# kopacja/rho2sdf.jl

Hardware: AMD Instinct MI355X
Metric: Mvoxels/s SDF extract on 512^3 grid over 100k HEX8; max|err| vs ref (higher is better)
Workload: dtype f64

## Files before the change

### rho2sdf.jl_amd/csrc/r2s_device_math.hpp

```cpp
#pragma once
#include <hip/hip_runtime.h>
#include <stdint.h>

namespace r2s {

#define R2S_DEV __device__ __forceinline__

struct alignas(16) ElemRec {
    double X[8][3];
    double r[8];
    double mn[3];
    double mx[3];
    double rmax;
    double rmin;
    double C[8][3];
    double Cr[8];
    double pn[6][3];
    double po[6];
    double pi[6];
    double nw[10];
};

struct alignas(16) BandItem {
    int32_t imin[3];
// ... 1309 lines not shown
    s.alpha *= 0.5;
    s.ls += 1;
    if (s.ls == 30) s.phase = FS_UPD;
}

template <class ER>
R2S_DEV void iso_full_upd(const ER& E, double rt, double rtol, IsoFullLane& s)
{
    s.Delta = (s.alpha < 1.0) ? ((s.alpha > 0.0) ? s.alpha * s.dmax : 0.25 * s.dmax) : fmin(2.0, fmax(s.Delta, 2.0 * s.dmax));
    if (s.stop == 2) {
        const bool near_feas = (fabs(s.c) <= 1e4 * rtol);
        double xr[3];
        if (!near_feas && s.nrest < R2S_ISO_MAX_RESTORE && iso_restore(E, s.x, rt, s.xi, s.c, xr)) {
            s.xi[0] = xr[0]; s.xi[1] = xr[1]; s.xi[2] = xr[2];
            s.mu = 0.0; s.Delta = 2.0; s.pat = 0; s.nrest++;
            s.it += 1;
            if (s.it == R2S_ISO_MAXIT) iso_full_fail(s); else s.phase = FS_EVAL;
            return;
        }
        iso_full_fail(s);
        return;
    }
    if (s.stop == 3 || s.stop == 4) { s.phase = FS_DONE; return; }
#pragma unroll
    for (int i = 0; i < 3; ++i) s.xi[i] = fmin(fmax(fma(s.alpha, s.d[i], s.xi[i]), -1.0), 1.0);
    if (s.stop == 1) { s.phase = FS_DONE; return; }
    s.it += 1;
    if (s.it == R2S_ISO_MAXIT) iso_full_fail(s); else s.phase = FS_EVAL;
}

#ifndef R2S_ISO_FAST_IT
#define R2S_ISO_FAST_IT 16
#endif
enum { ISO_IDLE = 0, ISO_EVAL, ISO_QP, ISO_FINISH, ISO_DONE, ISO_BAIL };

struct IsoLane {
    double x[3];
    double xi[3], mu, Delta;
    Sym3 H;
    double a[3], g[3], d[3];
    double se;
    double f, c, lam_new;
    int pat, it, p, step, phase;
    bool corner;
    bool seen;
};

R2S_DEV void iso_lane_bounds(const IsoLane& s, double lo[3], double hi[3])
{
#pragma unroll
    for (int i = 0; i < 3; ++i) {
        lo[i] = fmax(-1.0 - s.xi[i], -s.Delta);
        hi[i] = fmin(1.0 - s.xi[i], s.Delta);
    }
}

R2S_DEV void iso_lane_start(IsoLane& s, const double x[3])
{
    s.x[0] = x[0]; s.x[1] = x[1]; s.x[2] = x[2];
    s.xi[0] = s.xi[1] = s.xi[2] = 0.0;
    s.mu = 0.0; s.Delta = 2.0;
    s.pat = 0; s.it = 0;
    s.seen = false;
    s.phase = ISO_EVAL;
}

template <class ER>
R2S_DEV void iso_lane_eval(const ER& E, double rt, double rtol, IsoLane& s)
{
    double r[3], J[3][3], G[3][3], M2[3][3];
#pragma unroll
    for (int i = 0; i < 3; ++i) {
        const TriEval t = tri_eval_full(R2S_CX(E, i), s.xi);
        r[i] = s.x[i] - t.v;
        J[i][0] = t.d1; J[i][1] = t.d2; J[i][2] = t.d3;
        M2[i][0] = t.m12; M2[i][1] = t.m13; M2[i][2] = t.m23;
    }
    const double f = dot3(r[0], r[1], r[2], r[0], r[1], r[2]);
    const TriEval tr = tri_eval_full(R2S_CR(E), s.xi);
    double c = tr.v - rt;
    s.a[0] = tr.d1; s.a[1] = tr.d2; s.a[2] = tr.d3;
    if (fabs(c) <= rtol) c = 0.0;
#pragma unroll
    for (int j = 0; j < 3; ++j)
        if (fabs(s.a[j]) <= rtol) s.a[j] = 0.0;
#pragma unroll
    for (int j = 0; j < 3; ++j) s.g[j] = -2.0 * dot3(r[0], r[1], r[2], J[0][j], J[1][j], J[2][j]);
#pragma unroll
    for (int i = 0; i < 3; ++i)
#pragma unroll
        for (int j = i; j < 3; ++j)
            G[i][j] = G[j][i] = 2.0 * dot3(J[0][i], J[1][i], J[2][i], J[0][j], J[1][j], J[2][j]);
    s.pat = iso_clean_pattern(s.pat, s.xi);
    double lam;
    {
        double num = 0.0, den = 0.0;
        const int sp[3] = {s.pat & 3, (s.pat >> 2) & 3, s.pat >> 4};
#pragma unroll
        for (int i = 0; i < 3; ++i)
            if (!sp[i]) { num = fma(s.a[i], s.g[i], num); den = fma(s.a[i], s.a[i], den); }
        lam = (den > 0.0) ? -num / den : 0.0;
    }
    double S[3];
    {
        const double mr[3] = {tr.m12, tr.m13, tr.m23};
#pragma unroll
        for (int q = 0; q < 3; ++q)
            S[q] = fma(lam, mr[q], -2.0 * dot3(r[0], r[1], r[2], M2[0][q], M2[1][q], M2[2][q]));
    }
    double lo[3], hi[3];
    iso_lane_bounds(s, lo, hi);
    const double e = -c;
    double mplus = 0.0, mminus = 0.0;
// ... 35 lines not shown
    } else {
        double gp[3];
        iso_qp_data(G, S, s.a, s.g, sigma, e, s.H, gp);
        s.se = sigma * e;
        s.p = s.pat;
        s.step = 0;
        s.phase = iso_face_spd(s.H, s.pat) ? ISO_QP : ISO_BAIL;
    }
}

R2S_DEV void iso_lane_qp(IsoLane& s)
{
    QpOut o;
    double lo[3], hi[3], gp[3];
    iso_lane_bounds(s, lo, hi);
#pragma unroll
    for (int i = 0; i < 3; ++i) gp[i] = fma(-s.se, s.a[i], s.g[i]);
    const double e = -s.c;
    const int rc = qp_pattern(s.p, s.H, gp, s.a, e, lo, hi, o);
    if (rc == 1 && o.kkt) {
#pragma unroll
        for (int i = 0; i < 3; ++i) s.d[i] = fmin(fmax(o.d[i], lo[i]), hi[i]);
        s.lam_new = o.lam;
        s.phase = ISO_FINISH;
    } else if (rc == 0) {
        s.phase = ISO_BAIL;
    } else {
        s.p = o.next;
        s.step += 1;
        if (!(s.step < R2S_QP_WALK && s.p >= 0)) s.phase = ISO_BAIL;
    }
}

template <class ER>
R2S_DEV void iso_lane_finish(const ER& E, double rt, double rtol, IsoLane& s)
{
    const double dmax = fmax(fabs(s.d[0]), fmax(fabs(s.d[1]), fabs(s.d[2])));
    const bool near_feas = (fabs(s.c) <= 1e4 * rtol);
    if (!(dmax > R2S_ISO_TOL)) {
        if (s.corner && !near_feas) { s.phase = ISO_BAIL; return; }
    } else {
        const double ad = dot3(s.a[0], s.a[1], s.a[2], s.d[0], s.d[1], s.d[2]);
        const double pred_c = fabs(s.c) - fabs(s.c + ad);
        const double gd = dot3(s.g[0], s.g[1], s.g[2], s.d[0], s.d[1], s.d[2]);
        const double mu_keep = (fabs(s.c) <= 1e10 * rtol) ? 0.5 : 1.0;
        double mu_t = s.corner ? s.mu : fmax(mu_keep * s.mu, 2.0 * fabs(s.lam_new));
        if (s.corner && pred_c > 0.0) {
            const double need = 2.0 * fma(0.5, s.se, gd) / pred_c;
            if (need > mu_t) mu_t = need;
        }
        if (!(fma(-mu_t, pred_c, gd) < 0.0)) {
            if (pred_c > 0.0) mu_t = 2.0 * gd / pred_c;
            else {
                s.phase = (near_feas && !s.corner) ? ISO_DONE : ISO_BAIL;
                return;
            }
        }
        const double D = fma(-mu_t, pred_c, gd);
        const double phi0 = fma(mu_t, fabs(s.c), s.f);
        double xt[3], ft, ct;
#pragma unroll
        for (int i = 0; i < 3; ++i) xt[i] = fmin(fmax(fma(1.0, s.d[i], s.xi[i]), -1.0), 1.0);
        iso_eval_fc(E, s.x, rt, xt, ft, ct);
        if (!(fma(mu_t, fabs(ct), ft) <= fma(1e-4 * 1.0, D, phi0))) { s.phase = ISO_BAIL; return; }
        s.mu = mu_t;
        s.Delta = fmin(2.0, fmax(s.Delta, 2.0 * dmax));
        if (!s.corner) s.pat = s.p;
        s.seen = s.seen || (s.c == 0.0);
#pragma unroll
        for (int i = 0; i < 3; ++i) s.xi[i] = xt[i];
        s.it += 1;
        s.phase = (s.it == R2S_ISO_FAST_IT) ? ISO_BAIL : ISO_EVAL;
        return;
    }
    s.Delta = fmin(2.0, fmax(s.Delta, 2.0 * dmax));
#pragma unroll
    for (int i = 0; i < 3; ++i) s.xi[i] = fmin(fmax(fma(1.0, s.d[i], s.xi[i]), -1.0), 1.0);
    s.phase = ISO_DONE;
}

struct VoxState {
    double cur;
    double xp[3];
};

R2S_DEV bool write_value(VoxState& s, double d, const double xp[3], bool sym = false)
{
    if (sym && fabs(d) == s.cur) {
        const bool less = xp[0] < s.xp[0] || (xp[0] == s.xp[0] && (xp[1] < s.xp[1] || (xp[1] == s.xp[1] && xp[2] < s.xp[2])));
        if (less) { s.xp[0] = xp[0]; s.xp[1] = xp[1]; s.xp[2] = xp[2]; }
        return false;
    }
    if (fabs(d) < s.cur) {
        s.cur = d;
        s.xp[0] = xp[0]; s.xp[1] = xp[1]; s.xp[2] = xp[2];
        return true;
    }
    return false;
}

R2S_DEV bool projected_on_full_segment(VoxState& s, const ElemRec& E, double rt, const double xp[3],
                                       const double x[3], bool sym = false)
{
    double xi[3], N[8];
    inv_map_hex8(E, xp, xi);
// ... 391 lines not shown
```

### rho2sdf.jl_amd/csrc/rho2sdf_hip.hip

```cpp
#include <hip/hip_runtime.h>

#include <algorithm>
#include <cmath>
#include <cstdarg>
#include <cstddef>
#include <cstdio>
#include <cstring>
#include <initializer_list>
#include <utility>
#include <string>
#include <vector>

#include "../../include/rho2sdf_hip.h"
#include "r2s_common.hpp"
#include "r2s_device_math.hpp"

#include <type_traits>

using namespace r2s;

__constant__ int c_hex_isn[6][4] = {{0, 3, 2, 1}, {0, 1, 5, 4}, {1, 2, 6, 5},
                                    {2, 3, 7, 6}, {3, 0, 4, 7}, {4, 5, 6, 7}};

#define SCAN_BLOCK 256
// ... 1055 lines not shown
                    c = seg_end;
                    if (next >= v_end) continue;
                }
                if (s.phase == ISO_IDLE) {
                    const uint32_t v = next + __builtin_amdgcn_mbcnt_hi((uint32_t)(m_idle >> 32),
                                                  __builtin_amdgcn_mbcnt_lo((uint32_t)m_idle, 0u));
                    if (v < v_end) {
                        uint32_t li, lj, lk;
                        box_decode(dec, v, li, lj, lk);
                        const int i = lo0 + (int)li, j = lo1 + (int)lj, kl = lo2 + (int)lk;
                        double x[3];
                        x[0] = grid_coord(g, 0, i);
                        x[1] = grid_coord(g, 1, j);
                        x[2] = grid_coord(g, 2, slab_global_k(sl, kl));
                        iso_lane_start(s, x);
#ifdef R2S_ISO_STATS
                        dbg_trips = 0; dbg_qp = 0; dbg_ls = 0; dbg_el = items[it].el;
#endif
                        my = tile_slot(st_off, tb, i, j, kl);
                        eslot = cur_slot;
                    }
                }
                next += (uint32_t)__popcll(m_idle);
            }
            if (exhausted && __ballot(s.phase != ISO_IDLE) == 0) {
#ifdef R2S_ISO_WAVE_END
                if (lane == 0 && blockIdx.x < 4094) g_iso_wave_end[blockIdx.x] = wall_clock64();
#endif
                break;
            }
        }
        {
            const IsoElemLds& E = slots[eslot];
            ISO_STAT(0, s.phase == ISO_EVAL)
            if (s.phase == ISO_EVAL) iso_lane_eval(E, rho_t, E.rtol, s);
            ISO_STAT(1, s.phase == ISO_QP)
            if (s.phase == ISO_QP) iso_lane_qp(s);
            if (__popcll(__ballot(s.phase == ISO_QP)) >= R2S_ISO_QP2_MIN) {
                ISO_STAT(7, s.phase == ISO_QP)
                if (s.phase == ISO_QP) iso_lane_qp(s);
            }
            ISO_STAT(2, s.phase == ISO_FINISH)
            if (s.phase == ISO_FINISH) iso_lane_finish(E, rho_t, E.rtol, s);
            ISO_STAT(5, true)
#ifdef R2S_ISO_STATS
            if (s.phase != ISO_IDLE) dbg_trips += 1;
#endif
        }
    }
}

#ifdef R2S_STRAG_DIAG
__device__ unsigned long long g_strag_diag[3 * 16384];
extern "C" int r2s_debug_strag_diag(unsigned long long* out)
{
    if (hipMemcpyFromSymbol(out, HIP_SYMBOL(g_strag_diag), sizeof(unsigned long long) * 3 * 16384) != hipSuccess) return 1;
    static unsigned long long z[3 * 16384];
    return hipMemcpyToSymbol(HIP_SYMBOL(g_strag_diag), z, sizeof z) != hipSuccess;
}
__device__ unsigned long long g_strag_hist[256];
extern "C" int r2s_debug_strag_hist(unsigned long long* out)
{
    if (hipMemcpyFromSymbol(out, HIP_SYMBOL(g_strag_hist), sizeof(unsigned long long) * 256) != hipSuccess) return 1;
    static unsigned long long z[256];
    return hipMemcpyToSymbol(HIP_SYMBOL(g_strag_hist), z, sizeof z) != hipSuccess;
}
#endif
struct IsoCoefPad {
    double C[8][3];
    double Cr[8];
    double pad;
};
#ifndef R2S_STRAG_REFILL_MIN
#define R2S_STRAG_REFILL_MIN 8
#endif
#ifndef R2S_ENUM_COOP_MAX
// ... 457 lines not shown
    }
}

__global__ void __launch_bounds__(256) fill_kernel(double* __restrict__ p, int64_t n, double v)
{
    const int64_t stride = (int64_t)gridDim.x * blockDim.x;
    int64_t i = (int64_t)blockIdx.x * blockDim.x + threadIdx.x;
    const int64_t n2 = n >> 1;
    double2* p2 = reinterpret_cast<double2*>(p);
    const double2 vv = make_double2(v, v);
    for (int64_t j = i; j < n2; j += stride) p2[j] = vv;
    if (i == 0 && (n & 1)) p[n - 1] = v;
}

struct MainArgs {
    GridDev g;
    SlabInfo s;
    double rho_t;
    const uint32_t* active;
    uint32_t n_active;
    const uint32_t* band_off;
    const uint32_t* band_ent;
    const uint32_t* sign_off;
    const uint32_t* sign_ent;
    const BandItem* items;
    const void* erec;
    double* dist;
    double* sign;
    double* sdf;
    double* xp;
    const double* iso_res;
    const double* iso_res_xp;
    const void* sbox;
    const uint32_t* s_store_off;
    const double* sres;
    const uint8_t* hot;
    const uint32_t* abort_flag;
    int true_min;
    int sdf_mode;
};

template <class Rec, bool DO_DIST, bool DO_SIGN, bool TRI = true, bool SYM = false>
__global__ void __launch_bounds__(256) sdf_tiles_kernel(MainArgs A)
{
    const Rec* __restrict__ erec = static_cast<const Rec*>(A.erec);
    const uint32_t w = __builtin_amdgcn_readfirstlane((blockIdx.x * blockDim.x + threadIdx.x) >> 6);
    if (w >= A.n_active) return;
    const int lane = threadIdx.x & 63;
    const uint32_t ab = *A.abort_flag;
    const uint32_t t = A.active[w];
    if (ab) return;
    const int tx = t % A.s.ntx, ty = (t / A.s.ntx) % A.s.nty, tz = t / (A.s.ntx * A.s.nty);
    const int i = tx * 4 + (lane & 3), j = ty * 4 + ((lane >> 2) & 3), kl = tz * 4 + (lane >> 4);
    const int k = slab_global_k(A.s, kl);
    const bool valid = (i < A.g.nx) && (j < A.g.ny) && (kl < A.s.nzl) && (k < A.s.k1);
    double x[3];
    x[0] = grid_coord(A.g, 0, i);
    x[1] = grid_coord(A.g, 1, j);
    x[2] = grid_coord(A.g, 2, k);

    VoxState st;
    st.cur = 1.0e10;
    st.xp[0] = st.xp[1] = st.xp[2] = 0.0;
    if (DO_DIST) {
        const int ci = (int)cell_of(A.g, 0, x[0]), cj = (int)cell_of(A.g, 1, x[1]),
                  ck = (int)cell_of(A.g, 2, x[2]);
        const uint32_t b = A.band_off[t], e = A.band_off[t + 1];
// ... 47 lines not shown
                                if (A.iso_res_xp) {
                                    st.xp[0] = A.iso_res_xp[3 * slot[u]];
                                    st.xp[1] = A.iso_res_xp[3 * slot[u] + 1];
                                    st.xp[2] = A.iso_res_xp[3 * slot[u] + 2];
                                }
                            }
                        } else if constexpr (TRI) {
                            const BandItem& T = A.items[__builtin_amdgcn_readlane(my_it, (int)(q0 + u))];
                            process_triangle<Rec, SYM>(st, T, erec[T.el], A.rho_t, x);
                        }
                    }
                }
            }
        }
    }
    double sg = -1.0;
    if (DO_SIGN) {
        const uint32_t b = A.sign_off[t], e = A.sign_off[t + 1];
        if constexpr (std::is_same<Rec, ElemRec>::value) {
            if (A.hot[t]) {
                const SignBox* __restrict__ sbox = static_cast<const SignBox*>(A.sbox);
                bool any = false, done = false;
                double cmax = -INFINITY, max_local = 10.0;
                for (uint32_t p0 = b; p0 < e; p0 += 64u) {
                    const uint32_t n = (e - p0 < 64u) ? e - p0 : 64u;
                    int32_t hs[9];
#pragma unroll
                    for (int q = 0; q < 9; ++q) hs[q] = 0;
                    if ((uint32_t)lane < n) {
                        const uint32_t el = A.sign_ent[p0 + lane];
                        const int32_t* w = reinterpret_cast<const int32_t*>(&sbox[el]);
#pragma unroll
                        for (int q = 0; q < 8; ++q) hs[q] = w[q];
                        hs[8] = (int32_t)A.s_store_off[el];
                    }
                    for (uint32_t q0 = 0; q0 < n; q0 += 4u) {
                        bool in[4];
                        double v[4], rmax[4];
#pragma unroll
                        for (int u = 0; u < 4; ++u) {
                            const bool ok = q0 + u < n;
                            const int qq = (int)(ok ? q0 + u : n - 1u);
                            int32_t hh[9];
#pragma unroll
                            for (int q = 0; q < 9; ++q) hh[q] = __builtin_amdgcn_readlane(hs[q], qq);
                            const int32_t lo3[3] = {hh[0], hh[1], hh[2]}, dim3[3] = {hh[3], hh[4], hh[5]};
                            const uint32_t di = (uint32_t)(i - lo3[0]), dj = (uint32_t)(j - lo3[1]), dk = (uint32_t)(kl - lo3[2]);
                            in[u] = valid && ok && di < (uint32_t)dim3[0] && dj < (uint32_t)dim3[1] && dk < (uint32_t)dim3[2];
                            rmax[u] = __hiloint2double(hh[7], hh[6]);
                            v[u] = INFINITY;
                            if (in[u] && !done)
                                v[u] = A.sres[(size_t)tile_chunk((uint32_t)hh[8], tile_box(lo3, dim3), tx, ty, tz) * 64u + (uint32_t)lane];
                        }
#pragma unroll
                        for (int u = 0; u < 4; ++u) {
                            if (in[u]) {
                                any = true;
                                if (rmax[u] > cmax) cmax = rmax[u];
                                const double m = fabs(v[u]);
                                if (A.true_min) {
                                    if (m < 1.01 && !__builtin_signbit(v[u])) sg = 1.0;
                                } else if (!done && m < 1.01 && max_local > m) {
                                    if (!__builtin_signbit(v[u])) sg = 1.0;
                                    if (m < 0.95) done = true;
                                    else max_local = m;
                                }
                            }
// ... 128 lines not shown
    const int lane = threadIdx.x & 63;
    const int ntx = (nx + 3) / 4, nty = (ny + 3) / 4;
    const uint32_t t = ids[w];
    const int tx = t % ntx, ty = (t / ntx) % nty, tz = t / (ntx * nty);
    const int i = tx * 4 + (lane & 3), j = ty * 4 + ((lane >> 2) & 3), k = tz * 4 + (lane >> 4);
    if (i < nx && j < ny && k < nz) volume[((int64_t)k * ny + j) * nx + i] = payload[(size_t)w * 64 + lane];
}
__global__ void __launch_bounds__(256) unpack_segments_masks_kernel(const double* __restrict__ buf, int64_t seglen, uint32_t cap_full,
                                                                   uint32_t cap_mask, int nx, int ny, int nz, double magnitude,
                                                                   double* __restrict__ volume)
{
    const double* __restrict__ seg = buf + (int64_t)blockIdx.y * seglen;
    const int64_t nf = reinterpret_cast<const int64_t*>(seg)[0], nm = reinterpret_cast<const int64_t*>(seg)[1];
    const uint32_t w = __builtin_amdgcn_readfirstlane((blockIdx.x * blockDim.x + threadIdx.x) >> 6);
    if (nf < 0 || nf > (int64_t)cap_full || nm < 0 || nm > (int64_t)cap_mask || (int64_t)w >= nm) return;
    const uint64_t* __restrict__ masks = reinterpret_cast<const uint64_t*>(seg + 2 + (int64_t)cap_full * 64 + (cap_full + 1) / 2);
    const uint32_t* __restrict__ ids = reinterpret_cast<const uint32_t*>(masks + cap_mask);
    const int lane = threadIdx.x & 63;
    const int ntx = (nx + 3) / 4, nty = (ny + 3) / 4;
    const uint32_t t = ids[w];
    const int tx = t % ntx, ty = (t / ntx) % nty, tz = t / (ntx * nty);
    const int i = tx * 4 + (lane & 3), j = ty * 4 + ((lane >> 2) & 3), k = tz * 4 + (lane >> 4);
    if (i < nx && j < ny && k < nz) volume[((int64_t)k * ny + j) * nx + i] = ((masks[w] >> lane) & 1ull) ? magnitude : -magnitude;
}

struct r2s_plan {
    int device = 0;
    int n_cu = 256;
    DevBuf deg, ine_ptr, ine, cursor, erec, cls, fmask, nitems, item_off, items;
    DevBuf band_cnt, band_off, band_raw, band_ent, sign_cnt, sign_off, sign_raw, sign_ent;
    DevBuf active, active_sign, active_any, active_sonly, active_lean, active_tri, tri, hot, counters, scan_tmp[3], scan_tmp2[3], nchunks, chunk_off, iso_res, iso_res_xp, strag;
    DevBuf perm, wchunks, hardflag;
    DevBuf sbox, s_nchunks, s_chunk_off, sres;
    DevBuf nstore, store_off, s_nstore, s_store_off;
    SlabInfo last_s;
    GridDev last_g;
    uint32_t last_n_any = 0, last_n_band = 0, last_n_sonly = 0;
    bool has_last = false;
    uint32_t* h_pinned = nullptr;
    uint32_t* d_pinned = nullptr;
    struct Spec {
        bool valid = false;
        int64_t key[12] = {0};
        uint32_t v[16] = {0};
    } spec;
    hipEvent_t ev[8] = {nullptr, nullptr, nullptr, nullptr, nullptr, nullptr, nullptr, nullptr};
    hipStream_t st2 = nullptr;
    hipStream_t st3 = nullptr;
    hipEvent_t ev2[8] = {nullptr, nullptr, nullptr, nullptr, nullptr, nullptr, nullptr, nullptr};
    hipEvent_t ev_fast[2] = {nullptr, nullptr};
    bool fast_timed = false;
};

static int scan_exclusive2(r2s_plan* P, const uint32_t* in0, uint32_t* out0, const uint32_t* in1, uint32_t* out1,
                           int64_t n, hipStream_t st, int level = 0, int bank = 0)
{
    DevBuf* tmp = bank ? P->scan_tmp2 : P->scan_tmp;
    if (n <= 0) return 0;
    const unsigned ny = in1 ? 2u : 1u;
    const int64_t nb = (n + SCAN_TILE - 1) / SCAN_TILE;
    ScanPair sp;
    sp.in[0] = in0; sp.out[0] = out0; sp.in[1] = in1; sp.out[1] = out1;
    sp.sums[0] = sp.sums[1] = nullptr;
    if (nb == 1) {
        scan_block_kernel<<<dim3(1, ny), SCAN_BLOCK, 0, st>>>(sp, n);
        return 0;
    }
// ... 107 lines not shown
    int rc = check_device(device);
    if (rc) return rc;
    HIP_TRY(hipSetDevice(device));
    r2s_plan* P = new r2s_plan();
    P->device = device;
    {
        hipDeviceProp_t prop;
        if (hipGetDeviceProperties(&prop, device) == hipSuccess && prop.multiProcessorCount > 0) P->n_cu = prop.multiProcessorCount;
    }
    HIP_TRY(hipHostMalloc((void**)&P->h_pinned, 128, hipHostMallocMapped | hipHostMallocCoherent));
    HIP_TRY(hipHostGetDevicePointer((void**)&P->d_pinned, P->h_pinned, 0));
    for (int i = 0; i < 8; ++i) HIP_TRY(hipEventCreate(&P->ev[i]));
    for (int i = 0; i < 8; ++i) HIP_TRY(hipEventCreate(&P->ev2[i]));
    for (int i = 0; i < 2; ++i) HIP_TRY(hipEventCreate(&P->ev_fast[i]));
    {
        int prio_lo = 0, prio_hi = 0;
        HIP_TRY(hipDeviceGetStreamPriorityRange(&prio_lo, &prio_hi));
        (void)prio_lo;
        HIP_TRY(hipStreamCreateWithPriority(&P->st2, hipStreamNonBlocking, prio_hi));
        HIP_TRY(hipStreamCreateWithFlags(&P->st3, hipStreamNonBlocking));
    }
    *out = P;
    return 0;
}

void r2s_plan_destroy(r2s_plan* P)
{
    if (!P) return;
    (void)hipSetDevice(P->device);
    DevBuf* all[] = {&P->deg, &P->ine_ptr, &P->ine, &P->cursor, &P->erec, &P->cls, &P->fmask, &P->nitems,
                     &P->item_off, &P->items, &P->band_cnt, &P->band_off, &P->band_raw, &P->band_ent,
                     &P->sign_cnt, &P->sign_off, &P->sign_raw, &P->sign_ent, &P->active, &P->active_sign, &P->active_any, &P->active_sonly, &P->active_lean, &P->active_tri, &P->tri,
                     &P->hot, &P->counters, &P->nchunks, &P->chunk_off, &P->iso_res, &P->iso_res_xp, &P->strag,
                     &P->perm, &P->wchunks, &P->hardflag, &P->sbox, &P->s_nchunks, &P->s_chunk_off, &P->sres, &P->nstore, &P->store_off, &P->s_nstore, &P->s_store_off,
                     &P->scan_tmp[0], &P->scan_tmp[1], &P->scan_tmp[2], &P->scan_tmp2[0], &P->scan_tmp2[1], &P->scan_tmp2[2]};
    for (DevBuf* b : all) b->release();
    if (P->h_pinned) (void)hipHostFree(P->h_pinned);
    for (int i = 0; i < 8; ++i)
        if (P->ev[i]) (void)hipEventDestroy(P->ev[i]);
    for (int i = 0; i < 8; ++i)
        if (P->ev2[i]) (void)hipEventDestroy(P->ev2[i]);
    for (int i = 0; i < 2; ++i)
        if (P->ev_fast[i]) (void)hipEventDestroy(P->ev_fast[i]);
    if (P->st2) (void)hipStreamDestroy(P->st2);
    if (P->st3) (void)hipStreamDestroy(P->st3);
    delete P;
}


}

static uint32_t iso_straggler_cap(uint32_t n_store)
{
    static const int cap_env = getenv("R2S_ISO_STRAGGLER_CAP") ? atoi(getenv("R2S_ISO_STRAGGLER_CAP")) : 0;
    if (cap_env > 0) return (uint32_t)cap_env;
    const uint64_t slots = 64ull * std::max<uint32_t>(n_store, 1u);
    return (uint32_t)std::max<uint64_t>(slots / 16, std::min<uint64_t>(slots, 1ull << 20));
}

static int iso_project_hex(r2s_plan* P, hipStream_t st, uint32_t n_items, uint32_t n_chunks, uint32_t n_store, uint32_t wps,
                           const GridDev& g, const SlabInfo& s, double rho_t, double* res_xp, uint32_t* counters,
                           const uint32_t* abort_flag)
{
    static const int free_env = getenv("R2S_ISO_FREE") ? atoi(getenv("R2S_ISO_FREE")) : 0;
    const uint32_t resident = (uint32_t)P->n_cu * 4u * wps - (uint32_t)std::min(std::max(free_env, 0), (int)P->n_cu * 4);
    static const int group_env = getenv("R2S_ISO_GROUP") ? atoi(getenv("R2S_ISO_GROUP")) : 0;
    const uint32_t group = group_env > 0 ? (uint32_t)group_env
// ... 128 lines not shown
    HIP_TRY(hipEventRecord(P->ev2[5], st));
    HIP_TRY(hipStreamWaitEvent(P->st2, P->ev2[0], 0));
    {
        const int64_t n = nel * ET::NEN;
        node_degree_kernel<<<(unsigned)((n + 255) / 256), 256, 0, P->st2>>>(dIEN, nel, ET::NEN, nnp, P->deg.as<uint32_t>(), (int*)counters);
        int rc = scan_exclusive(P, P->deg.as<uint32_t>(), P->ine_ptr.as<uint32_t>(), nnp + 1, P->st2);
        if (rc) return rc;
        ine_fill_kernel<<<(unsigned)((n + 255) / 256), 256, 0, P->st2>>>(dIEN, nel, ET::NEN, nnp, P->ine_ptr.as<uint32_t>(), P->cursor.as<uint32_t>(), P->ine.as<uint32_t>());
    }
    HIP_TRY(hipEventRecord(P->ev2[1], P->st2));
    if constexpr (std::is_same<typename ET::Rec, ElemRec>::value) {
        HIP_TRY(hipStreamWaitEvent(P->st2, P->ev2[5], 0));
        HIP_TRY(hipStreamWaitEvent(P->st3, P->ev2[5], 0));
        static const int no_inner_env = getenv("R2S_SIGN_NO_INNER") ? atoi(getenv("R2S_SIGN_NO_INNER")) : 0;
        hex_planes_kernel<<<(unsigned)((nel * 6 + 255) / 256), 256, 0, P->st3>>>(P->erec.as<ElemRec>(), nel,
                                                                                 (no_inner_env || prm.sign_no_inner) ? 1 : 0);
        HIP_TRY(hipEventRecord(P->ev2[5], P->st3));
    }
    constexpr bool HEX = std::is_same<typename ET::Rec, ElemRec>::value;
    const double rmax_needed = HEX ? -INFINITY : rho_t - 1e-12 * (fabs(rho_t) + 1.0);
    const bool sign_items = HEX && want_sign && nel > 0;
    ReadBack rb2;
    if constexpr (HEX) {
        if (sign_items) {
            zero_many(P->st2, {{P->sign_cnt.p, sizeof(uint32_t) * (size_t)(ntiles + 1)}, {P->hot.p, (size_t)ntiles + 1}});
            sign_hot_kernel<ElemRec><<<(unsigned)((nel * BIN_LANES + 255) / 256), 256, 0, P->st2>>>(P->erec.as<ElemRec>(), (uint32_t)nel, g, s, rho_t, P->hot.as<uint8_t>());
            sign_bin_kernel<ElemRec, false><<<(unsigned)((nel * BIN_LANES + 255) / 256), 256, 0, P->st2>>>(P->erec.as<ElemRec>(), (uint32_t)nel, g, s, P->sign_cnt.as<uint32_t>(), nullptr, nullptr, P->hot.as<uint8_t>(), abort_flag, rmax_needed);
            int rc = scan_exclusive2(P, P->sign_cnt.as<uint32_t>(), P->sign_off.as<uint32_t>(), nullptr, nullptr, (int64_t)ntiles + 1, P->st2, 0, 1);
            if (rc) return rc;
            ENSURE(P->sbox, sizeof(SignBox) * (size_t)nel);
            ENSURE(P->s_nchunks, sizeof(uint32_t) * (size_t)(nel + 1));
            ENSURE(P->s_chunk_off, sizeof(uint32_t) * (size_t)(nel + 1));
            ENSURE(P->s_nstore, sizeof(uint32_t) * (size_t)(nel + 1));
            ENSURE(P->s_store_off, sizeof(uint32_t) * (size_t)(nel + 1));
            zero_many(P->st2, {{P->s_nchunks.p, sizeof(uint32_t) * (size_t)(nel + 1)}, {P->s_nstore.p, sizeof(uint32_t) * (size_t)(nel + 1)}});
            sign_box_kernel<<<(unsigned)((nel * BIN_LANES + 255) / 256), 256, 0, P->st2>>>(P->erec.as<ElemRec>(), (uint32_t)nel, g, s, P->hot.as<uint8_t>(), P->sbox.as<SignBox>(), P->s_nchunks.as<uint32_t>(), P->s_nstore.as<uint32_t>());
            rc = scan_exclusive2(P, P->s_nchunks.as<uint32_t>(), P->s_chunk_off.as<uint32_t>(), P->s_nstore.as<uint32_t>(),
                                 P->s_store_off.as<uint32_t>(), nel + 1, P->st2, 0, 1);
            if (rc) return rc;
            rb2.add(P->s_chunk_off.as<uint32_t>() + nel, 1, 11);
            rb2.add(P->s_store_off.as<uint32_t>() + nel, 1, 13);
            HIP_TRY(hipEventRecord(P->ev2[7], P->st2));
        }
    }
    HIP_TRY(hipStreamWaitEvent(st, P->ev2[1], 0));
    face_mask_kernel<ET><<<(unsigned)((nel * ET::NES + 255) / 256), 256, 0, st>>>(
        dIEN, nel, P->ine_ptr.as<uint32_t>(), P->ine.as<uint32_t>(), P->cls.as<uint8_t>(), P->fmask.as<uint32_t>(),
        P->nitems.as<uint32_t>(), (const int*)counters);
    {
        int rc = scan_exclusive(P, P->nitems.as<uint32_t>(), P->item_off.as<uint32_t>(), nel + 1, st);
        if (rc) return rc;
    }
    {
        ReadBack rb;
        rb.add(P->item_off.as<uint32_t>() + nel, 1, 0);
        rb.add(counters, 1, 1);
        read_back_kernel<<<1, 64, 0, st>>>(rb, P->d_pinned, ex, counters + 15);
    }
    if (!spec) {
        HIP_TRY(hipStreamSynchronize(st));
        if (P->h_pinned[1]) return fail(R2S_ERR_ARG, "IEN contains node ids outside 1..nnp");
        cnt[0] = P->h_pinned[0];
        cnt[1] = 0;
    }
    const uint32_t n_items = want_dist ? cnt[0] : 0;
    ENSURE(P->items, sizeof(BandItem) * (size_t)std::max<uint32_t>(n_items, 1));
    ENSURE(P->nchunks, sizeof(uint32_t) * (size_t)(n_items + 1));
    ENSURE(P->chunk_off, sizeof(uint32_t) * (size_t)(n_items + 1));
    ENSURE(P->nstore, sizeof(uint32_t) * (size_t)(n_items + 1));
    ENSURE(P->store_off, sizeof(uint32_t) * (size_t)(n_items + 1));
    if (n_items) {
        ENSURE(P->hardflag, (size_t)n_items + 1);
        zero_many(st, {{P->nchunks.p, sizeof(uint32_t) * (size_t)(n_items + 1)}, {P->nstore.p, sizeof(uint32_t) * (size_t)(n_items + 1)},
                       {P->hardflag.p, (size_t)n_items + 1}});
// ... 120 lines not shown
        if (cnt[7] > 64u)
            bin_sort_kernel<<<(n_active_sign + 3) / 4, 256, 0, bs>>>(P->active_sign.as<uint32_t>(), n_active_sign, P->sign_off.as<uint32_t>(), P->sign_raw.as<uint32_t>(), P->sign_ent.as<uint32_t>(), abort_flag);
    }
    HIP_TRY(hipEventRecord(P->ev[2], bs));

    static const bool overlap_env = !(getenv("R2S_NO_OVERLAP") && atoi(getenv("R2S_NO_OVERLAP")));
    const bool overlap = !HEX && overlap_env && mode == R2S_OUT_SDF && want_sign && want_dist;
    const bool fork = HEX && overlap_env && want_sign && want_dist && n_chunks && n_schunks;
    {
        const bool two_streams = overlap || fork;
        hipStream_t fs = two_streams ? P->st2 : st;
        const unsigned fill_grid = 256 * 8;
        if (two_streams) HIP_TRY(hipStreamWaitEvent(P->st2, P->ev[2], 0));
        HIP_TRY(hipEventRecord(P->ev2[0], fs));
        if (mode & R2S_OUT_DIST) fill_kernel<<<fill_grid, 256, 0, fs>>>(d_dist, nvox, 1.0e10);
        if (mode & R2S_OUT_SIGN) fill_kernel<<<fill_grid, 256, 0, fs>>>(d_sign, nvox, -1.0);
        if (mode & R2S_OUT_SDF) fill_kernel<<<fill_grid, 256, 0, fs>>>(d_sdf, nvox, -1.0e10);
        if (mode & R2S_OUT_XP) HIP_TRY(hipMemsetAsync(d_xp, 0, sizeof(double) * 3 * (size_t)nvox, fs));
        HIP_TRY(hipEventRecord(P->ev2[3], fs));
        HIP_TRY(hipEventRecord(P->ev[3], st));
        if (two_streams) HIP_TRY(hipEventRecord(P->ev2[1], P->st2));
    }

    {
        MainArgs A;
        A.g = g; A.s = s; A.rho_t = rho_t;
        A.true_min = prm.true_min ? 1 : 0;
        A.band_off = P->band_off.as<uint32_t>(); A.band_ent = P->band_ent.as<uint32_t>();
        A.sign_off = P->sign_off.as<uint32_t>(); A.sign_ent = P->sign_ent.as<uint32_t>();
        A.items = P->items.as<BandItem>(); A.erec = P->erec.as<typename ET::Rec>();
        A.dist = (mode & R2S_OUT_DIST) ? d_dist : nullptr;
        A.sign = (mode & R2S_OUT_SIGN) ? d_sign : nullptr;
        A.sdf = (mode & R2S_OUT_SDF) ? d_sdf : nullptr;
        A.sbox = P->sbox.p; A.s_store_off = P->s_store_off.as<uint32_t>(); A.sres = P->sres.as<double>();
        A.hot = P->hot.as<uint8_t>();
        A.abort_flag = abort_flag;
        if constexpr (HEX) {
            hipStream_t ss = fork ? P->st2 : st;
            if (!fork) HIP_TRY(hipEventRecord(P->ev2[1], ss));
            if (want_sign && n_schunks) {
                const uint32_t cpw = 8, nwaves = (n_schunks + cpw - 1) / cpw;
                HIP_TRY(hipStreamWaitEvent(ss, P->ev2[5], 0));
                sign_project_kernel<<<nwaves, 64, 0, ss>>>(P->sbox.as<SignBox>(), (uint32_t)nel, P->s_chunk_off.as<uint32_t>(), n_schunks, P->s_store_off.as<uint32_t>(), cpw,
                                                          P->erec.as<ElemRec>(), g, s, rho_t, P->hot.as<uint8_t>(), P->sres.as<double>(), abort_flag);
            }
            HIP_TRY(hipEventRecord(P->ev2[4], ss));
            A.xp = (mode & R2S_OUT_XP) ? d_xp : nullptr;
            A.sdf_mode = 1;
            const uint32_t n_sonly = cnt[9];
            const bool early_sign_tiles = want_dist && want_sign && !(mode & R2S_OUT_XP);
            if (early_sign_tiles && n_sonly) {
                MainArgs B = A;
                B.active = P->active_sonly.as<uint32_t>(); B.n_active = n_sonly;
                sdf_tiles_kernel<ElemRec, false, true><<<n_sonly, 64, 0, ss>>>(B);
            }
            HIP_TRY(hipEventRecord(P->ev2[2], ss));
            A.iso_res = P->iso_res.as<double>();
            A.iso_res_xp = (mode & R2S_OUT_XP) ? P->iso_res_xp.as<double>() : nullptr;
            if (!early_iso) HIP_TRY(hipEventRecord(P->ev[7], st));
            if (want_dist && n_chunks && !early_iso) {
                static const int wps_env = getenv("R2S_ISO_WPS") ? atoi(getenv("R2S_ISO_WPS")) : 0;
                const uint32_t wps = (wps_env >= 1 && wps_env <= 3) ? (uint32_t)wps_env : 3u;
                if (fork) HIP_TRY(hipStreamWaitEvent(st, P->ev2[0], 0));
                double* const res_xp = (mode & R2S_OUT_XP) ? P->iso_res_xp.as<double>() : nullptr;
                { const int rc = iso_project_hex(P, st, n_items, n_chunks, n_store, wps, g, s, rho_t, res_xp, counters, abort_flag); if (rc) return rc; }
            }
            if (!early_iso) HIP_TRY(hipEventRecord(P->ev[6], st));
            if (fork) HIP_TRY(hipStreamWaitEvent(st, P->ev2[4], 0));
            if (want_dist && want_sign && early_sign_tiles) {
                const uint32_t n_lean = cnt[14], n_tri = cnt[15];
                if (n_lean) {
                    A.active = P->active_lean.as<uint32_t>(); A.n_active = n_lean;
                    sdf_tiles_kernel<ElemRec, true, true, false><<<n_lean, 64, 0, st>>>(A);
                }
                if (n_tri) {
                    A.active = P->active_tri.as<uint32_t>(); A.n_active = n_tri;
// ... 237 lines not shown
```

Before: 33380.

## Reuse line-search trial evaluation as next iteration's full eval in iso solver

The trial-point evaluation is moved out of the finish phase into a new TRIAL phase. It shares one full trilinear evaluation (values and derivatives) with the next EVAL phase, so an accepted trial point is not re-evaluated. Lane state now uses unions to hold the trial data without growing registers. This also turns the finish step's inline divergent evaluation into a wave-uniform phase, but trials that are rejected now pay for a full derivative evaluation instead of only f and c. A field is also renamed (s_store_off to sgn_store_off).

```diff
diff --git a/rho2sdf.jl_amd/csrc/r2s_device_math.hpp b/rho2sdf.jl_amd/csrc/r2s_device_math.hpp
--- a/rho2sdf.jl_amd/csrc/r2s_device_math.hpp
+++ b/rho2sdf.jl_amd/csrc/r2s_device_math.hpp
@@ -1365,15 +1365,18 @@
 #ifndef R2S_ISO_FAST_IT
 #define R2S_ISO_FAST_IT 16
 #endif
-enum { ISO_IDLE = 0, ISO_EVAL, ISO_QP, ISO_FINISH, ISO_DONE, ISO_BAIL };
+enum { ISO_IDLE = 0, ISO_EVAL, ISO_QP, ISO_FINISH, ISO_DONE, ISO_BAIL, ISO_TRIAL };
 
 struct IsoLane {
     double x[3];
     double xi[3], mu, Delta;
     Sym3 H;
-    double a[3], g[3], d[3];
-    double se;
-    double f, c, lam_new;
+    double a[3], g[3];
+    union { double d[3]; double xt[3]; };
+    union { double se; double mu_t; };
+    union { double f; double phi_t; };
+    union { double lam_new; double Delta_t; };
+    double c;
     int pat, it, p, step, phase;
     bool corner;
     bool seen;
@@ -1392,26 +1395,56 @@
 {
     s.x[0] = x[0]; s.x[1] = x[1]; s.x[2] = x[2];
     s.xi[0] = s.xi[1] = s.xi[2] = 0.0;
+    s.xt[0] = s.xt[1] = s.xt[2] = 0.0;
     s.mu = 0.0; s.Delta = 2.0;
     s.pat = 0; s.it = 0;
     s.seen = false;
     s.phase = ISO_EVAL;
 }
 
+struct IsoVals {
+    TriEval t[3], tr;
+    double r[3], f, c;
+};
 template <class ER>
-R2S_DEV void iso_lane_eval(const ER& E, double rt, double rtol, IsoLane& s)
-{
-    double r[3], J[3][3], G[3][3], M2[3][3];
+R2S_DEV void iso_lane_values(const ER& E, double rt, const IsoLane& s, IsoVals& v)
+{
 #pragma unroll
     for (int i = 0; i < 3; ++i) {
-        const TriEval t = tri_eval_full(R2S_CX(E, i), s.xi);
-        r[i] = s.x[i] - t.v;
+        v.t[i] = tri_eval_full(R2S_CX(E, i), s.xt);
+        v.r[i] = s.x[i] - v.t[i].v;
+    }
+    v.f = dot3(v.r[0], v.r[1], v.r[2], v.r[0], v.r[1], v.r[2]);
+    v.tr = tri_eval_full(R2S_CR(E), s.xt);
+    v.c = v.tr.v - rt;
+}
+
+R2S_DEV void iso_lane_accept(IsoLane& s, const IsoVals& v)
+{
+    if (!(fma(s.mu_t, fabs(v.c), v.f) <= s.phi_t)) { s.phase = ISO_BAIL; return; }
+    s.mu = s.mu_t;
+    s.Delta = s.Delta_t;
+    if (!s.corner) s.pat = s.p;
+    s.seen = s.seen || (s.c == 0.0);
+#pragma unroll
+    for (int i = 0; i < 3; ++i) s.xi[i] = s.xt[i];
+    s.it += 1;
+    s.phase = (s.it == R2S_ISO_FAST_IT) ? ISO_BAIL : ISO_EVAL;
+}
+
+R2S_DEV void iso_lane_eval(double rtol, IsoLane& s, const IsoVals& v)
+{
+    double J[3][3], G[3][3], M2[3][3];
+    const double* r = v.r;
+#pragma unroll
+    for (int i = 0; i < 3; ++i) {
+        const TriEval& t = v.t[i];
         J[i][0] = t.d1; J[i][1] = t.d2; J[i][2] = t.d3;
         M2[i][0] = t.m12; M2[i][1] = t.m13; M2[i][2] = t.m23;
     }
-    const double f = dot3(r[0], r[1], r[2], r[0], r[1], r[2]);
-    const TriEval tr = tri_eval_full(R2S_CR(E), s.xi);
-    double c = tr.v - rt;
+    const double f = v.f;
+    const TriEval& tr = v.tr;
+    double c = v.c;
     s.a[0] = tr.d1; s.a[1] = tr.d2; s.a[2] = tr.d3;
     if (fabs(c) <= rtol) c = 0.0;
 #pragma unroll
@@ -1513,8 +1546,7 @@
     }
 }
 
-template <class ER>
-R2S_DEV void iso_lane_finish(const ER& E, double rt, double rtol, IsoLane& s)
+R2S_DEV void iso_lane_finish(double rtol, IsoLane& s)
 {
     const double dmax = fmax(fabs(s.d[0]), fmax(fabs(s.d[1]), fabs(s.d[2])));
     const bool near_feas = (fabs(s.c) <= 1e4 * rtol);
@@ -1539,19 +1571,12 @@
         }
         const double D = fma(-mu_t, pred_c, gd);
         const double phi0 = fma(mu_t, fabs(s.c), s.f);
-        double xt[3], ft, ct;
-#pragma unroll
-        for (int i = 0; i < 3; ++i) xt[i] = fmin(fmax(fma(1.0, s.d[i], s.xi[i]), -1.0), 1.0);
-        iso_eval_fc(E, s.x, rt, xt, ft, ct);
-        if (!(fma(mu_t, fabs(ct), ft) <= fma(1e-4 * 1.0, D, phi0))) { s.phase = ISO_BAIL; return; }
-        s.mu = mu_t;
-        s.Delta = fmin(2.0, fmax(s.Delta, 2.0 * dmax));
-        if (!s.corner) s.pat = s.p;
-        s.seen = s.seen || (s.c == 0.0);
-#pragma unroll
-        for (int i = 0; i < 3; ++i) s.xi[i] = xt[i];
-        s.it += 1;
-        s.phase = (s.it == R2S_ISO_FAST_IT) ? ISO_BAIL : ISO_EVAL;
+        s.phi_t = fma(1e-4 * 1.0, D, phi0);
+        s.mu_t = mu_t;
+        s.Delta_t = fmin(2.0, fmax(s.Delta, 2.0 * dmax));
+#pragma unroll
+        for (int i = 0; i < 3; ++i) s.xt[i] = fmin(fmax(fma(1.0, s.d[i], s.xi[i]), -1.0), 1.0);
+        s.phase = ISO_TRIAL;
         return;
     }
     s.Delta = fmin(2.0, fmax(s.Delta, 2.0 * dmax));
diff --git a/rho2sdf.jl_amd/csrc/rho2sdf_hip.hip b/rho2sdf.jl_amd/csrc/rho2sdf_hip.hip
--- a/rho2sdf.jl_amd/csrc/rho2sdf_hip.hip
+++ b/rho2sdf.jl_amd/csrc/rho2sdf_hip.hip
@@ -1111,8 +1111,13 @@
         }
         {
             const IsoElemLds& E = slots[eslot];
-            ISO_STAT(0, s.phase == ISO_EVAL)
-            if (s.phase == ISO_EVAL) iso_lane_eval(E, rho_t, E.rtol, s);
+            ISO_STAT(0, s.phase == ISO_TRIAL || s.phase == ISO_EVAL)
+            if (s.phase == ISO_TRIAL || s.phase == ISO_EVAL) {
+                IsoVals v;
+                iso_lane_values(E, rho_t, s, v);
+                if (s.phase == ISO_TRIAL) iso_lane_accept(s, v);
+                if (s.phase == ISO_EVAL) iso_lane_eval(E.rtol, s, v);
+            }
             ISO_STAT(1, s.phase == ISO_QP)
             if (s.phase == ISO_QP) iso_lane_qp(s);
             if (__popcll(__ballot(s.phase == ISO_QP)) >= R2S_ISO_QP2_MIN) {
@@ -1120,7 +1125,7 @@
                 if (s.phase == ISO_QP) iso_lane_qp(s);
             }
             ISO_STAT(2, s.phase == ISO_FINISH)
-            if (s.phase == ISO_FINISH) iso_lane_finish(E, rho_t, E.rtol, s);
+            if (s.phase == ISO_FINISH) iso_lane_finish(E.rtol, s);
             ISO_STAT(5, true)
 #ifdef R2S_ISO_STATS
             if (s.phase != ISO_IDLE) dbg_trips += 1;
@@ -1644,7 +1649,7 @@
     const double* iso_res;
     const double* iso_res_xp;
     const void* sbox;
-    const uint32_t* s_store_off;
+    const uint32_t* sgn_store_off;
     const double* sres;
     const uint8_t* hot;
     const uint32_t* abort_flag;
@@ -1758,7 +1763,7 @@
                         const int32_t* w = reinterpret_cast<const int32_t*>(&sbox[el]);
 #pragma unroll
                         for (int q = 0; q < 8; ++q) hs[q] = w[q];
-                        hs[8] = (int32_t)A.s_store_off[el];
+                        hs[8] = (int32_t)A.sgn_store_off[el];
                     }
                     for (uint32_t q0 = 0; q0 < n; q0 += 4u) {
                         bool in[4];
@@ -1953,7 +1958,7 @@
     DevBuf active, active_sign, active_any, active_sonly, active_lean, active_tri, tri, hot, counters, scan_tmp[3], scan_tmp2[3], nchunks, chunk_off, iso_res, iso_res_xp, strag;
     DevBuf perm, wchunks, hardflag;
     DevBuf sbox, s_nchunks, s_chunk_off, sres;
-    DevBuf nstore, store_off, s_nstore, s_store_off;
+    DevBuf nstore, store_off, s_nstore, sgn_store_off;
     SlabInfo last_s;
     GridDev last_g;
     uint32_t last_n_any = 0, last_n_band = 0, last_n_sonly = 0;
@@ -2127,7 +2132,7 @@
                      &P->item_off, &P->items, &P->band_cnt, &P->band_off, &P->band_raw, &P->band_ent,
                      &P->sign_cnt, &P->sign_off, &P->sign_raw, &P->sign_ent, &P->active, &P->active_sign, &P->active_any, &P->active_sonly, &P->active_lean, &P->active_tri, &P->tri,
                      &P->hot, &P->counters, &P->nchunks, &P->chunk_off, &P->iso_res, &P->iso_res_xp, &P->strag,
-                     &P->perm, &P->wchunks, &P->hardflag, &P->sbox, &P->s_nchunks, &P->s_chunk_off, &P->sres, &P->nstore, &P->store_off, &P->s_nstore, &P->s_store_off,
+                     &P->perm, &P->wchunks, &P->hardflag, &P->sbox, &P->s_nchunks, &P->s_chunk_off, &P->sres, &P->nstore, &P->store_off, &P->s_nstore, &P->sgn_store_off,
                      &P->scan_tmp[0], &P->scan_tmp[1], &P->scan_tmp[2], &P->scan_tmp2[0], &P->scan_tmp2[1], &P->scan_tmp2[2]};
     for (DevBuf* b : all) b->release();
     if (P->h_pinned) (void)hipHostFree(P->h_pinned);
@@ -2322,14 +2327,14 @@
             ENSURE(P->s_nchunks, sizeof(uint32_t) * (size_t)(nel + 1));
             ENSURE(P->s_chunk_off, sizeof(uint32_t) * (size_t)(nel + 1));
             ENSURE(P->s_nstore, sizeof(uint32_t) * (size_t)(nel + 1));
-            ENSURE(P->s_store_off, sizeof(uint32_t) * (size_t)(nel + 1));
+            ENSURE(P->sgn_store_off, sizeof(uint32_t) * (size_t)(nel + 1));
             zero_many(P->st2, {{P->s_nchunks.p, sizeof(uint32_t) * (size_t)(nel + 1)}, {P->s_nstore.p, sizeof(uint32_t) * (size_t)(nel + 1)}});
             sign_box_kernel<<<(unsigned)((nel * BIN_LANES + 255) / 256), 256, 0, P->st2>>>(P->erec.as<ElemRec>(), (uint32_t)nel, g, s, P->hot.as<uint8_t>(), P->sbox.as<SignBox>(), P->s_nchunks.as<uint32_t>(), P->s_nstore.as<uint32_t>());
             rc = scan_exclusive2(P, P->s_nchunks.as<uint32_t>(), P->s_chunk_off.as<uint32_t>(), P->s_nstore.as<uint32_t>(),
-                                 P->s_store_off.as<uint32_t>(), nel + 1, P->st2, 0, 1);
+                                 P->sgn_store_off.as<uint32_t>(), nel + 1, P->st2, 0, 1);
             if (rc) return rc;
             rb2.add(P->s_chunk_off.as<uint32_t>() + nel, 1, 11);
-            rb2.add(P->s_store_off.as<uint32_t>() + nel, 1, 13);
+            rb2.add(P->sgn_store_off.as<uint32_t>() + nel, 1, 13);
             HIP_TRY(hipEventRecord(P->ev2[7], P->st2));
         }
     }
@@ -2516,7 +2521,7 @@
         A.dist = (mode & R2S_OUT_DIST) ? d_dist : nullptr;
         A.sign = (mode & R2S_OUT_SIGN) ? d_sign : nullptr;
         A.sdf = (mode & R2S_OUT_SDF) ? d_sdf : nullptr;
-        A.sbox = P->sbox.p; A.s_store_off = P->s_store_off.as<uint32_t>(); A.sres = P->sres.as<double>();
+        A.sbox = P->sbox.p; A.sgn_store_off = P->sgn_store_off.as<uint32_t>(); A.sres = P->sres.as<double>();
         A.hot = P->hot.as<uint8_t>();
         A.abort_flag = abort_flag;
         if constexpr (HEX) {
@@ -2525,7 +2530,7 @@
             if (want_sign && n_schunks) {
                 const uint32_t cpw = 8, nwaves = (n_schunks + cpw - 1) / cpw;
                 HIP_TRY(hipStreamWaitEvent(ss, P->ev2[5], 0));
-                sign_project_kernel<<<nwaves, 64, 0, ss>>>(P->sbox.as<SignBox>(), (uint32_t)nel, P->s_chunk_off.as<uint32_t>(), n_schunks, P->s_store_off.as<uint32_t>(), cpw,
+                sign_project_kernel<<<nwaves, 64, 0, ss>>>(P->sbox.as<SignBox>(), (uint32_t)nel, P->s_chunk_off.as<uint32_t>(), n_schunks, P->sgn_store_off.as<uint32_t>(), cpw,
                                                           P->erec.as<ElemRec>(), g, s, rho_t, P->hot.as<uint8_t>(), P->sres.as<double>(), abort_flag);
             }
             HIP_TRY(hipEventRecord(P->ev2[4], ss));
```

Result: no change. 33880 (median of 6 runs) (+1.5%).
